# Xingskcs/Distributed-TensorFlow-Examples

Measured on AMD Instinct MI355X. Metric: images/sec (whole node), MNIST CNN sync all-reduce, higher is better.
Workload: dtype bf16; 1 GPU; model=mnist_cnn (conv5x5x32-pool-conv5x5x64-pool-fc1024-dropout-fc10, 3274634 params), global_batch=1024, parallelism=dp1, per_gpu_batch=1024, optimizer=adam (TF1), hip_graph=True, steps_per_graph=4, join_deferred=True, distinct_gpus=1, grad_allreduce=none (1 rank), ranks_seen_by_comm=1

## Files before the change

csrc/bindings/torch_ops.cpp:

```cpp
#include <ATen/ATen.h>
#include <ATen/hip/HIPContext.h>
#include <torch/custom_class.h>
#include <torch/library.h>
#include <algorithm>
#include <cmath>
#include <cstring>
#include <vector>

#include "../kernels/augment.h"
#include "../kernels/conv.h"
#include "../kernels/conv_f32.h"
#include "../kernels/imgconv.h"
#include "../kernels/norm.h"
#include "../kernels/elementwise.h"
#include "../kernels/eval.h"
#include "../kernels/gemm_dense.h"
#include "../kernels/head.h"
#include "../kernels/lstm_seq.h"
#include "../kernels/gradnorm.h"
#include "../kernels/optim.h"
#include "opt_state.h"

using at::Tensor;
using c10::optional;
// ... 271 lines not shown
  a.w = reinterpret_cast<const dtfe::bf16*>(w.data_ptr());
  a.bias = ptr_or_null<float>(bias);
  a.act = (int)act; a.pool = pool;
  a.y = reinterpret_cast<dtfe::bf16*>(y.data_ptr());
  a.argmax = ptr_or_null<uint8_t>(argmax);
  a.relu_mask = ptr_or_null<dtfe::bf16>(relu_mask);
  TORCH_CHECK(w.numel() == N * KH * KW * CS, "imgconv: weight size");
  TORCH_CHECK(y.numel() == B * OH * OW * N / (pool ? 4 : 1), "imgconv: output size");
  a.tstamp = tstamp.has_value() && tstamp->defined() ? reinterpret_cast<uint64_t*>(tstamp->data_ptr()) : nullptr;
  a.bns = bn_src_of(bn_src, (long)B * SH * SW, CS, bn_eps, bn_momentum, bn_save);
  TORCH_CHECK(!a.bns.stats || a.src, "imgconv: BN-on-load needs a plain source");
  a.sc_src = ptr_or_null<dtfe::bf16>(sc_src);
  if (a.sc_src) {
    TORCH_CHECK(sc_stride >= 1 && OH % sc_stride == 0 && OW % sc_stride == 0 && sc_src->dim() == 4 &&
                    sc_src->size(0) == B && sc_src->size(1) == OH / sc_stride && sc_src->size(2) == OW / sc_stride &&
                    sc_src->size(3) >= N,
                "imgconv: shortcut gradient [B][OH/s][OW/s][>= N]");
    a.sc_stride = (int)sc_stride;
    a.sc_C = (int)sc_src->size(3);
  }
  return dtfe::launch_imgconv(a, cur_stream());
}

void conv1_gather_fwd(const Tensor& images, const Tensor& labels_src, int64_t seed, const Tensor& counter,
                      const Tensor& done, const Tensor& labels_dst, const Tensor& x, const Tensor& w,
                      const optional<Tensor>& bias, const Tensor& y, const Tensor& argmax, at::TensorList zero) {
  check_cuda(images, "images");
  TORCH_CHECK(images.scalar_type() == at::kByte && images.dim() == 2 && images.size(1) == 784,
              "conv1_gather_fwd: uint8 [rows][784] dataset");
  TORCH_CHECK(x.scalar_type() == at::kBFloat16 && x.numel() % 784 == 0, "conv1_gather_fwd: bf16 x [B][28][28]");
  dtfe::ImgConvArgs a{};
  a.B = (int)(x.numel() / 784); a.SH = a.SW = 28; a.CS = 1; a.OH = a.OW = 28; a.N = 32;
  a.KH = a.KW = 5; a.stride = 1; a.pad = 2; a.dil = 1;
  a.src = reinterpret_cast<const dtfe::bf16*>(x.data_ptr());
  a.w = reinterpret_cast<const dtfe::bf16*>(w.data_ptr());
  a.bias = ptr_or_null<float>(bias);
  a.act = dtfe::ACT_RELU; a.pool = 1;
  a.y = reinterpret_cast<dtfe::bf16*>(y.data_ptr());
  a.argmax = reinterpret_cast<uint8_t*>(argmax.data_ptr());
  TORCH_CHECK(w.numel() == 32 * 25 && y.numel() == (int64_t)a.B * 14 * 14 * 32 && argmax.numel() == y.numel(),
              "conv1_gather_fwd: MNIST conv1 shapes");
  a.g_src = images.data_ptr<uint8_t>(); a.g_rows = images.size(0); a.g_seed = (uint64_t)seed;
  a.g_counter = counter.data_ptr<int64_t>();
  a.g_done = done.numel() ? reinterpret_cast<uint32_t*>(done.data_ptr()) : nullptr;
  a.g_labels_src = labels_src.data_ptr<int32_t>(); a.g_labels_dst = labels_dst.data_ptr<int32_t>();
  TORCH_CHECK(zero.size() <= 4, "conv1_gather_fwd: at most 4 zero ranges");
  for (const Tensor& z : zero) {
    TORCH_CHECK(z.is_contiguous() && (z.numel() * z.element_size()) % 4 == 0, "conv1_gather_fwd: zero ranges");
    a.zptr[a.nz] = reinterpret_cast<uint32_t*>(z.data_ptr());
    a.zlen[a.nz++] = (long)(z.numel() * z.element_size() / 4);
  }
  TORCH_CHECK(dtfe::launch_conv1_copies_fwd(a, cur_stream()), "conv1_gather_fwd: needs B >= 256");
}

std::vector<int64_t> imgwgrad(const Tensor& src, const optional<Tensor>& dy, const optional<Tensor>& dy_pooled,
                              const optional<Tensor>& dy_argmax, const Tensor& dw, const optional<Tensor>& db,
                              int64_t B, int64_t SH, int64_t SW, int64_t CS, int64_t OH, int64_t OW, int64_t N,
                              int64_t KH, int64_t KW, int64_t stride, int64_t pad, double scale,
                              const optional<Tensor>& ws, int64_t max_blocks, const optional<at::TensorList>& bn_src,
                              double bn_eps, bool defer) {
  check_cuda(src, "src");
  dtfe::ImgWgradArgs a{};
  a.defer_reduce = defer ? 1 : 0;
  a.bns = bn_src_of(bn_src, (long)B * SH * SW, CS, bn_eps, 0.0, false);
  a.max_blocks = (int)max_blocks;
  if (ws.has_value() && ws->defined()) {
    TORCH_CHECK(ws->scalar_type() == at::kFloat && ws->numel() >= dtfe::imgwgrad_ws_floats((int)N, (int)(KH * KW * CS)),
                "imgwgrad: workspace too small (ops.wgrad_ws_floats)");
    a.ws = ws->data_ptr<float>();
  }
  a.B = (int)B; a.SH = (int)SH; a.SW = (int)SW; a.CS = (int)CS; a.OH = (int)OH; a.OW = (int)OW; a.N = (int)N;
  a.KH = (int)KH; a.KW = (int)KW; a.stride = (int)stride; a.pad = (int)pad;
  a.src = reinterpret_cast<const dtfe::bf16*>(src.data_ptr());
  a.dy = ptr_or_null<dtfe::bf16>(dy);
  a.dy_pooled = ptr_or_null<dtfe::bf16>(dy_pooled);
// ... 1076 lines not shown
                  y.size(2) == (x.size(2) + 1) / 2, "bn_relu_pool3: y bf16 / am uint8 [B][ceil(H/2)][ceil(W/2)][C]");
  dtfe::BnArgs a = bn_common(x, stats, 1);
  a.gamma = gamma.data_ptr<float>();
  a.beta = beta.data_ptr<float>();
  a.mean = ptr_or_null<float>(mean);
  a.invstd = ptr_or_null<float>(invstd);
  a.moving_mean = ptr_or_null<float>(moving_mean);
  a.moving_var = ptr_or_null<float>(moving_var);
  a.eps = (float)eps; a.momentum = (float)momentum;
  dtfe::launch_bn_relu_pool3(a, reinterpret_cast<dtfe::bf16*>(y.data_ptr()), am.data_ptr<uint8_t>(), (int)x.size(0),
                             (int)x.size(1), (int)x.size(2), (int)y.size(1), (int)y.size(2), cur_stream());
}

void maxpool3_bwd(const Tensor& dy, const Tensor& am, const Tensor& dx) {
  dtfe::launch_maxpool3_bwd(reinterpret_cast<const dtfe::bf16*>(dy.data_ptr()), am.data_ptr<uint8_t>(),
                            reinterpret_cast<dtfe::bf16*>(dx.data_ptr()), (int)dx.size(0), (int)dx.size(1),
                            (int)dx.size(2), (int)dx.size(3), (int)dy.size(1), (int)dy.size(2), cur_stream());
}

TORCH_LIBRARY(dtfe, m) {
  m.def("conv1_gather_fwd(Tensor images, Tensor labels_src, int seed, Tensor(a!) counter, Tensor(b!) done,"
        " Tensor(c!) labels_dst, Tensor(d!) x, Tensor w, Tensor? bias, Tensor(e!) y, Tensor(f!) argmax,"
        " Tensor(g!)[] zero) -> ()");
  m.def("lstm_seq_fwd(Tensor(a!) xh, Tensor K, Tensor bias, float forget_bias, Tensor(b!) act, Tensor(c!) c,"
        " Tensor(d!) hT, Tensor? xsrc=None, Tensor? ysrc=None, Tensor(e!)? ydst=None, Tensor(f!)? zero0=None,"
        " Tensor(g!)? zero1=None) -> bool");
  m.def("lstm_seq_bwd(Tensor K, Tensor act, Tensor c, Tensor dhT, Tensor(a!) dg, int I, Tensor? dl=None,"
        " Tensor? wo=None) -> bool");
  m.def("lstm_status(bool reset=False) -> int", &lstm_status);
  m.def("lstm_last_split() -> int", &lstm_last_split);
  m.def("bn_stats(Tensor x, Tensor(a!) stats) -> ()");
  m.def("bn_infer(Tensor x, Tensor gamma, Tensor beta, Tensor moving_mean, Tensor moving_var, float eps, int act,"
        " Tensor? res, int rstride, int OH, int OW, Tensor(a!) out) -> ()");
  m.def("bn_apply(Tensor x, Tensor stats, Tensor gamma, Tensor beta, Tensor(a!)? mean, Tensor(b!)? invstd,"
        " Tensor(c!)? moving_mean, Tensor(d!)? moving_var, float eps, float momentum, int act, Tensor? res,"
        " int rstride, int OH, int OW, Tensor(e!) out, Tensor(f!)? mask_out=None, Tensor(g!)[]? res_bn=None) -> ()");
  m.def("bn_bwd_stats(Tensor dy, Tensor? y, Tensor x, Tensor mean, Tensor invstd, Tensor(a!) stats, int act,"
        " Tensor? gamma=None, Tensor? beta=None, Tensor(b!)[]? res_bn=None) -> ()");
  m.def("bn_bwd_apply(Tensor dy, Tensor? y, Tensor x, Tensor mean, Tensor invstd, Tensor gamma, Tensor stats,"
        " int act, Tensor(a!) dx, Tensor(b!)? dres, Tensor(c!)? dgamma, Tensor(d!)? dbeta, Tensor? beta=None) -> ()");
  m.def("shortcut_grad_add(Tensor g, Tensor(a!) dx, int stride) -> ()");
  m.def("gap_fwd(Tensor x, Tensor(a!) y) -> ()");
  m.def("gap_bwd(Tensor dy, Tensor(a!) dx) -> ()");
  m.def("maxpool3_fwd(Tensor x, Tensor(a!) y, Tensor(b!) am) -> ()");
  m.def("maxpool3_bwd(Tensor dy, Tensor am, Tensor(a!) dx) -> ()");
  m.def("bn_relu_pool3(Tensor x, Tensor stats, Tensor gamma, Tensor beta, Tensor(a!)? mean, Tensor(b!)? invstd,"
// ... 84 lines not shown
      " Tensor(b!)? loss_rows, Tensor(c!)? loss_sum, Tensor(d!)? correct, Tensor(e!)? probs) -> ()");
  m.def(
      "gan_loss(Tensor d_real, Tensor d_fake, Tensor(a!) gen_loss, Tensor(b!) disc_loss, Tensor(c!) dz_real_disc,"
      " Tensor(d!) dz_fake_disc, Tensor(e!) dz_fake_gen, float clamp_eps) -> ()");
  m.def("gan_disc_head(Tensor d1, Tensor w, Tensor? b, Tensor(a!)? p, Tensor(b!)? dlog, Tensor(c!)? dlog_g,"
        " Tensor(d!) gw, Tensor(e!)? gb, Tensor(f!) dd1, Tensor(g!) ddf, Tensor(h!) gen_loss, Tensor(i!) disc_loss,"
        " Tensor(j!) ws, float clamp_eps=0.0) -> bool");
  m.def("gan_head_ws_floats(int B, int DH) -> int");
  m.def("epoch_signal(Tensor(a!) ctr) -> ()");
  m.def("mse_sigmoid(Tensor y, Tensor t, Tensor(a!) loss, Tensor(b!) dz, Tensor(c!)? ws=None) -> ()");
  m.def("colsum(Tensor x, int M, int N, int ld, Tensor(a!) db, float scale) -> ()");
  m.def("unpool_f32(Tensor g, Tensor argmax, Tensor(a!) out, int B, int PH, int PW, int C) -> ()");
  m.def("head_xent_f32(Tensor h, Tensor w, Tensor? b, Tensor labels, Tensor(a!) dz, Tensor(b!) dl, Tensor(c!) loss_sum,"
        " Tensor(d!) correct, Tensor(e!)? logits, float scale, float inv_keep, Tensor(f!)? step_counter) -> bool");
  m.def("conv1_wgrad_pooled_f32(Tensor dp, Tensor argmax, Tensor x, Tensor(a!) dw, Tensor(b!)? db, Tensor(c!) ws,"
        " int B, int H, int W, int K, float scale) -> bool");
  m.def("transpose_taps_f32(Tensor input, Tensor(a!) out, int O, int T, int C) -> ()");
  m.def("act_grad(Tensor dy, Tensor y, Tensor(a!) dz, int act) -> ()");
  m.def("bias_act(Tensor x, Tensor? bias, Tensor(a!) out, int act, float keep, int seed, Tensor? counter) -> ()");
}

TORCH_LIBRARY_IMPL(dtfe, CUDA, m) {
  m.impl("conv1_gather_fwd", &conv1_gather_fwd);
  m.impl("lstm_seq_fwd", &lstm_seq_fwd);
  m.impl("lstm_seq_bwd", &lstm_seq_bwd);
  m.impl("bn_stats", &bn_stats);
  m.impl("bn_apply", &bn_apply);
  m.impl("bn_infer", &bn_infer);
  m.impl("bn_bwd_stats", &bn_bwd_stats);
  m.impl("bn_bwd_apply", &bn_bwd_apply);
  m.impl("shortcut_grad_add", &shortcut_grad_add);
  m.impl("gap_fwd", &gap_fwd);
  m.impl("gap_bwd", &gap_bwd);
  m.impl("maxpool3_fwd", &maxpool3_fwd);
  m.impl("maxpool3_bwd", &maxpool3_bwd);
  m.impl("bn_relu_pool3", &bn_relu_pool3);
  m.impl("pool3_bn_bwd", &pool3_bn_bwd);
  m.impl("gemm", &gemm);
  m.impl("conv_fwd", &conv_fwd);
  m.impl("conv_dgrad", &conv_dgrad);
  m.impl("conv_wgrad", &conv_wgrad);
  m.impl("head_xent", &head_xent);
  m.impl("head_wgrad", &head_wgrad);
  m.impl("grad_sumsq", &grad_sumsq);
  m.impl("scale_", &scale_);
  m.impl("eval_metrics", &eval_metrics);
// ... 33 lines not shown
```

csrc/kernels/imgconv.h:

```cpp
#pragma once
#include "bn_chan.h"
#include "common.h"

namespace dtfe {

struct ImgConvArgs {
  int B, SH, SW, CS;
  int OH, OW, N;
  int KH, KW, stride, pad;
  int flip_taps;
  int dil;
  const bf16* src;
  const bf16* src_pooled;
  const uint8_t* src_argmax;
  const bf16* w;
  const float* bias;
  int act, pool;
  bf16* y;
  uint8_t* argmax;
  const bf16* relu_mask;
  const uint8_t* g_src;
  long g_rows;
  uint64_t g_seed;
  int64_t* g_counter;
// ... 19 lines not shown
  int imgs_per_block;
  float* ws;
  int max_blocks;
  int diag;
  BnSrc bns;
  int defer_reduce;
};

struct WpReduceItem {
  const float* ws; float* dw; float* db; float scale; int nblk, plen, MT, CTW, KC, N;
};
constexpr int WP_GROUP_MAX = 32;
void launch_wgrad_reduce_group(const WpReduceItem* it, int n, hipStream_t s);

bool imgconv_supported(int SH, int SW, int CS, int N, int KH, int KW, int stride, int pad);
bool launch_imgconv(const ImgConvArgs& a, hipStream_t s);
bool launch_imgconv_persistent(const ImgConvArgs& a, hipStream_t s, bool* sc_done = nullptr);
bool imgwgrad_supported(const ImgWgradArgs& a);
long imgwgrad_ws_floats(int N, int KC);
void launch_imgwgrad(const ImgWgradArgs& a, hipStream_t s, WpReduceItem& deferred);
bool launch_imgwgrad_persistent(const ImgWgradArgs& a, hipStream_t s, WpReduceItem& deferred);
bool launch_conv1_copies_fwd(const ImgConvArgs& a, hipStream_t s);
bool launch_conv1_copies_wgrad(const ImgWgradArgs& a, hipStream_t s);


void launch_partials_reduce(const float* ws, int nblk, int len, int nw, float* dw, float* db, float scale,
                            hipStream_t s);


__device__ __forceinline__ void unpool4(const u32x4_t pv, const u32x2_t am, u32x4_t (&out)[4]) {
#pragma unroll
  for (int h = 0; h < 2; ++h) {
    const uint32_t lo = am[h] & 0x01010101u, hi = (am[h] >> 1) & 0x01010101u;
    const uint32_t m[4] = {((lo | hi) ^ 0x01010101u) * 0xFFu, (lo & ~hi) * 0xFFu, (hi & ~lo) * 0xFFu,
                           (lo & hi) * 0xFFu};
#pragma unroll
    for (int q = 0; q < 4; ++q) {
      out[q][2 * h] = pv[2 * h] & __builtin_amdgcn_perm(0u, m[q], 0x01010000u);
      out[q][2 * h + 1] = pv[2 * h + 1] & __builtin_amdgcn_perm(0u, m[q], 0x03030202u);
    }
  }
}

}
```

csrc/kernels/imgconv1_copies.hip:

```cpp
#include "imgconv.h"

#include <stdexcept>
#include <type_traits>

namespace dtfe {

namespace {

constexpr int TH = 256;
constexpr int HI = 28;
constexpr int PWD = 48, PRW = 32;
constexpr int CWD = 40;
constexpr int CSZ = PRW * CWD + 8;
constexpr int NCH = 32;
constexpr int XCH = HI * HI / 4;

__device__ __forceinline__ u32x4_t ld16l(const bf16* p) { return *reinterpret_cast<const u32x4_t*>(p); }

template <int B, int E, typename F>
__device__ __forceinline__ void static_for_c1(F&& f) {
  if constexpr (B < E) {
    f(std::integral_constant<int, B>{});
    static_for_c1<B + 1, E>(f);
  }
}

__device__ __forceinline__ void load_img(const bf16* x, long b, u32x2_t& v) {
  if (threadIdx.x < XCH) v = *reinterpret_cast<const u32x2_t*>(x + b * (HI * HI) + threadIdx.x * 4);
}
__device__ __forceinline__ void write_img(bf16* P, const u32x2_t& v) {
  if (threadIdx.x < XCH) {
    const int r = threadIdx.x / 7, c = (threadIdx.x - r * 7) * 4;
    *reinterpret_cast<u32x2_t*>(P + (r + 2) * PWD + c + 4) = v;
  }
}

__device__ __forceinline__ uint32_t shr16(uint32_t lo, uint32_t hi) {
  return (uint32_t)((((uint64_t)hi << 32) | lo) >> 16);
}
template <int S>
__device__ __forceinline__ void build_copies(const bf16* P, bf16* C) {
  constexpr int HALF = (S + 1) / 2;
  const int t = threadIdx.x & 127, r = t >> 2, c8 = (t & 3) * 8;
  const u32x4_t* src = reinterpret_cast<const u32x4_t*>(P + r * PWD + c8);
  uint32_t d[12];
#pragma unroll
  for (int j = 0; j < 3; ++j) {
    const u32x4_t v = src[j];
#pragma unroll
    for (int e = 0; e < 4; ++e) d[4 * j + e] = v[e];
  }
  auto emit = [&](auto sc) {
    constexpr int s = decltype(sc)::value;
    constexpr int e0 = s + 2;
    u32x4_t o;
#pragma unroll
    for (int j = 0; j < 4; ++j) o[j] = (e0 & 1) ? shr16(d[(e0 >> 1) + j], d[(e0 >> 1) + j + 1]) : d[(e0 >> 1) + j];
    *reinterpret_cast<u32x4_t*>(C + s * CSZ + r * CWD + c8) = o;
  };
  if (threadIdx.x < 128) {
    static_for_c1<0, HALF>(emit);
  } else {
    static_for_c1<HALF, S>(emit);
  }
}

template <int ACT>
__global__ __launch_bounds__(TH) void conv1c_fwd_kernel(ImgConvArgs a) {
  __shared__ __attribute__((aligned(16))) bf16 P[PRW * PWD];
  __shared__ __attribute__((aligned(16))) bf16 C[8 * CSZ];
  const int lane = threadIdx.x & 63, wid = threadIdx.x >> 6, g = lane >> 4;
  for (int i = threadIdx.x; i < PRW * PWD / 8; i += TH) reinterpret_cast<u32x4_t*>(P)[i] = u32x4_t{0u, 0u, 0u, 0u};

  bf16x8_t bw[2][2];
  float biasv[2];
#pragma unroll
  for (int nt = 0; nt < 2; ++nt) {
    const int n = nt * 16 + (lane & 15);
    biasv[nt] = a.bias ? a.bias[n] : 0.f;
#pragma unroll
    for (int st = 0; st < 2; ++st) {
      const int kh = st == 0 ? g : 4;
      const bool rowok = st == 0 || g == 0;
      s16x8_t v;
#pragma unroll
      for (int j = 0; j < 8; ++j) v[j] = (short)((rowok && j < 5) ? a.w[n * 25 + kh * 5 + j] : 0);
      bw[nt][st] = __builtin_bit_cast(bf16x8_t, v);
    }
  }

  const int64_t gstep = a.g_src ? *a.g_counter : 0;
  for (int z = 0; z < ((a.diag & 8) ? 0 : a.nz); ++z)
    for (long i = (long)blockIdx.x * TH + threadIdx.x; i < a.zlen[z]; i += (long)gridDim.x * TH) a.zptr[z][i] = 0u;
  auto load = [&](long bb, u32x2_t& v) {
    if (!a.g_src) {
      load_img(a.src, bb, v);
      return;
    }
    const long r = (long)(hash_u32(a.g_seed, (uint64_t)gstep * a.B + bb) % (uint32_t)a.g_rows);
    if (threadIdx.x < XCH) {
      const uint32_t px = *reinterpret_cast<const uint32_t*>(a.g_src + r * (HI * HI) + threadIdx.x * 4);
      const float k = 1.f / 255.f;
      v = u32x2_t{pack_bf16x2((float)(px & 0xffu) * k, (float)((px >> 8) & 0xffu) * k),
                  pack_bf16x2((float)((px >> 16) & 0xffu) * k, (float)(px >> 24) * k)};
      *reinterpret_cast<u32x2_t*>(const_cast<bf16*>(a.src) + bb * (HI * HI) + threadIdx.x * 4) = v;
    }
    if (threadIdx.x == 0 && a.g_labels_dst) a.g_labels_dst[bb] = a.g_labels_src[r];
  };
  u32x2_t xv = {0u, 0u};
  long b = blockIdx.x;
  if (b < a.B) load(b, xv);
  __syncthreads();
  for (; b < a.B; b += gridDim.x) {
    write_img(P, xv);
    __syncthreads();
    if (b + gridDim.x < a.B) load(b + gridDim.x, xv);
    if (!(a.diag & 2)) build_copies<8>(P, C);
    __syncthreads();
    for (int t = wid; t < ((a.diag & 4) ? 0 : 49); t += 4) {
      const int m = t * 16 + (lane & 15), q = m & 3, w = m >> 2;
      const int oy = 2 * (w / 14) + (q >> 1), ox = 2 * (w % 14) + (q & 1);
      const int s = ox & 7;
      const bf16* ab = C + s * CSZ + (ox - s) + oy * CWD;
      const bf16x8_t a0 = __builtin_bit_cast(bf16x8_t, ld16l(ab + g * CWD));
      const bf16x8_t a1 = __builtin_bit_cast(bf16x8_t, ld16l(ab + 4 * CWD));
      f32x4_t acc[2];
#pragma unroll
// ... 197 lines not shown
```

distributed-tensorflow-examples_amd/models/mnist_cnn.py:

```python
from __future__ import annotations

import contextlib

import torch

from .. import ops
from ..optim import FlatParams, Optimizer, OptimizerConfig, VarSpec
from .base import ModelDef, ScaledScalar, StepProgram

IMG, C1, C2, FC, NCLS = 28, 32, 64, 1024, 10
KS = 5


def _normal(std):
    return lambda shape, g: torch.randn(*shape, generator=g) * std


def _zeros(shape, g):
    return torch.zeros(*shape)


def _conv_to_tf(t):
    return t.permute(1, 2, 3, 0).contiguous()

# ... 94 lines not shown
        self.data_ctr = torch.zeros(1, dtype=torch.int64, device=d)
        self.data_done = torch.zeros(1, dtype=torch.int32, device=d)
        self.no_done = torch.zeros(0, dtype=torch.int32, device=d)
        self.g1 = dict(B=B, H=IMG, W=IMG, C=1, Cout=C1, OH=IMG, OW=IMG, KH=KS, KW=KS, stride=1, pad=2)
        self.g2 = dict(B=B, H=14, W=14, C=C1, Cout=C2, OH=14, OW=14, KH=KS, KW=KS, stride=1, pad=2)
        self.ic1 = dict(B=B, SH=IMG, SW=IMG, CS=1, OH=IMG, OW=IMG, N=C1, KH=KS, KW=KS, stride=1, pad=2)
        self.ic2 = dict(B=B, SH=14, SW=14, CS=C1, OH=14, OW=14, N=C2, KH=KS, KW=KS, stride=1, pad=2)
        self.ic2_dgrad = dict(B=B, SH=14, SW=14, CS=C2, OH=14, OW=14, N=C1, KH=KS, KW=KS, stride=1, pad=KS - 1 - 2)
        n = self.names
        P = self.P
        self.w = {k: P.w16[n[k]] for k in ("wc1", "wc2", "wd1", "out")}
        self.wt = {"wc2": P.wt16[n["wc2"]]}
        self.b = {k: P.view(n[k]) for k in ("bc1", "bc2", "bd1", "bout")}
        self.gw = {k: P.gview(n[k]) for k in ("wc1", "wc2", "wd1", "out", "bc1", "bc2", "bd1", "bout")}
        lo1, hi1 = P.range_of([n["out"], n["bout"], n["bd1"], n["wd1"]])
        lo2, hi2 = P.range_of([n["wc2"], n["bc2"], n["wc1"], n["bc1"]])
        self.buckets = [(lo1, hi1), (lo2, hi2)]
        ra = P.range_of([n["out"], n["bout"]])
        rc = P.range_of([n["wc2"], n["bc2"], n["wc1"], n["bc1"]])
        self.accum = [P.grad[ra[0]:ra[1]], P.grad[rc[0]:rc[1]], self.loss_sum, self.correct]
        self.par = self.device.type == "cuda"
        self.c2_blocks = 192
        self.fused_gather = True
        self.late_split = True
        K1 = 7 * 7 * C2
        self.t_fwd = self._glds_tile(self.p2, P.w16[n["wd1"]], B, FC, K1, K1, K1, 19)
        self.t_dgrad = (self._glds_tile(self.dzf, P.w16[n["wd1"]], B, K1, FC, FC, K1, ops.FC_TILE, bmode=ops.RMAJ)
                        or self._glds_tile(self.dzf, P.w16[n["wd1"]], B, K1, FC, FC, K1, 12))
        self.t_wgrad = (self._glds_tile(self.dzf, self.p2, FC, K1 + 1, B, FC, K1, ops.FC_TILE, b_ones_row=K1,
                                        bmode=ops.RMAJ)
                        or self._glds_tile(self.dzf, self.p2, FC, K1 + 1, B, FC, K1, 12, b_ones_row=K1))
        if (self.t_dgrad == ops.FC_TILE) != (self.t_wgrad == ops.FC_TILE):
            self.t_dgrad = self._glds_tile(self.dzf, P.w16[n["wd1"]], B, K1, FC, FC, K1, 12)
            self.t_wgrad = self._glds_tile(self.dzf, self.p2, FC, K1 + 1, B, FC, K1, 12, b_ones_row=K1)
        self.head_gemm = batch > 1024
        self.head_parts = None if self.head_gemm else torch.zeros(2 * ((B + 3) // 4), device=d, dtype=torch.float32)
        self.head_splits = max(1, min(16, B // 128))
        bm, bn = ops.TILE_DIMS[4]
        ntiles = -(-NCLS // bm) * -(-(FC + 1) // bn)
        self.ws_head = (torch.empty(self.head_splits * ntiles * bm * bn, device=d, dtype=torch.float32),
                        torch.zeros(ntiles, device=d, dtype=torch.int32)) if self.head_gemm else None
        self.opt_fc = self.opt_conv = None
        self._late = None
        self.schedule = []
        self.logits = None
        if self.par:
            self.s_c2 = torch.cuda.Stream(device=d)
            self.ws_c2 = torch.empty(ops.wgrad_ws_floats(C2, KS * KS * C1), device=d, dtype=torch.float32)
            self.c2_done = torch.zeros(1, device=d, dtype=torch.int32)
            self.c2_seen = torch.zeros(1, device=d, dtype=torch.int32)
        self.defer_join = False
        self._pending_join = False

    def _glds_tile(self, A, Bm, M, N, K, lda, ldb, tile, b_ones_row=-1, bmode=ops.KMAJ):
        if self.device.type == "cuda" and ops.glds_ok(A, Bm, M, N, K, tile, lda, ldb, b_ones_row=b_ones_row,
                                                      bmode=bmode):
            return tile
        return None

    def forward(self, keep=None, logits=None):
        B = self.B
        keep = self.keep if keep is None else keep
        if self.data is not None and self.device.type == "cuda" and B >= 256 and self.fused_gather:
            ops.require().conv1_gather_fwd(self.data.images, self.data.labels, self.seed + 1, self.data_ctr,
                                           self.no_done, self.labels, self.x, self.w["wc1"], self.b["bc1"],
                                           self.p1, self.a1, self.accum)
        else:
            if self.data is not None:
                ops.gather_rows(self.data.images, self.x.view(B, -1), None, self.data.labels, self.labels,
                                seed=self.seed + 1, counter=self.data_ctr, done=None, zero=self.accum)
            else:
                for t in self.accum:
                    t.zero_()
            ops.imgconv(self.w["wc1"], self.p1, src=self.x, bias=self.b["bc1"], argmax=self.a1, act=ops.ACT_RELU,
                        pool=True, **self.ic1)
        ops.imgconv(self.w["wc2"], self.p2, src=self.p1, bias=self.b["bc2"], argmax=self.a2, act=ops.ACT_RELU,
                    pool=True, **self.ic2)
        K1 = 7 * 7 * C2
        ops.gemm(self.p2, self.w["wd1"], self.h, M=B, N=FC, K=K1, bias=self.b["bd1"], act=ops.ACT_RELU,
                 keep=keep, seed=self.seed + 2, counter=self.data_ctr, tile=self.t_fwd)
        ops.head_xent(self.h, self.w["out"], self.b["bout"], self.labels, self.dzf, self.dl, self.loss_sum,
                      self.correct, logits, scale=1.0 / B, inv_keep=1.0 / keep,
                      step_counter=self.data_ctr if self.data is not None else None,
                      parts=self.head_parts)

    def forward_backward(self):
        B = self.B
        K1 = 7 * 7 * C2
        self.schedule = []
        self.forward()
        main = torch.cuda.current_stream(self.device) if self.par else None
        with ops.gemm_group(self.dzf) as grp:
            self._head_wgrad(grp)
            self._fc1_dgrad(B, K1, grp)
            self._fc1_wgrad(B, K1, grp)
        if self.allreduce is not None:
            self.allreduce.launch(0)
            self.schedule.append("allreduce:0")
        if self.par:
            self.s_c2.wait_stream(main)
# ... 269 lines not shown
```

distributed-tensorflow-examples_amd/ops/__init__.py:

```python
from __future__ import annotations

import contextlib
import functools
import math
import os

import numpy as np
import torch

from ._lib import (ACT_CODES, ACT_NONE, ACT_RELU, ACT_SIGMOID, ACT_TANH, KMAJ, OPT_ADAM, OPT_MOMENTUM,
                   OPT_RMSPROP, OPT_SGD, RMAJ, available, load, require)

__all__ = [
    "gemm", "linear_fwd", "conv_fwd", "conv_dgrad", "conv_wgrad", "head_xent", "apply_gradients", "apply_gradients_group", "opt_state",
    "gather_rows", "uniform_fill", "cast_", "softmax_xent", "gan_loss", "mse_sigmoid", "colsum", "act_grad",
    "bias_act", "ACT_NONE", "ACT_RELU", "ACT_SIGMOID", "ACT_TANH", "ACT_CODES", "KMAJ", "RMAJ", "OPT_SGD",
    "OPT_MOMENTUM", "OPT_ADAM", "OPT_RMSPROP", "available", "load", "require", "pick_tile", "split_workspace",
    "TILE_DIMS", "FC_TILE", "TILE_SMALL", "GEMM_KTILE", "GLDS_TILES", "glds_ok", "ones_page", "bn_stats", "bn_apply", "bn_bwd_stats",
    "bn_bwd_apply", "relu_bits", "shortcut_grad_add",
    "gap_fwd", "gap_bwd", "gemm_group", "seq_stage", "wgrad_tallk", "tallk_ws_floats", "maxpool3_fwd", "maxpool3_bwd", "bn_relu_pool3", "pool3_bn_bwd", "imgconv", "imgwgrad", "hash_u32", "hash_uniform",
    "imgconv_shortcut", "dense_head", "WgradReduces", "conv1_wgrad_pooled_f32",
    "head_xent_f32", "gan_disc_head", "gan_head_ws_floats", "epoch_signal", "grad_norm_plan", "grad_sumsq", "scale_",
    "augment_rows", "augment_draws", "AUG_SALT", "epoch_permutation", "shuffled_rows", "SHUF_SALT", "lr_schedule_spec", "lr_schedule_value", "lr_schedule_pack",
    "eval_metrics", "eval_state", "eval_state_dict", "eval_rows_ref",
# ... 374 lines not shown
        sd = torch.zeros(B, SH * dil, SW * dil, CS)
        sd[:, ::dil, ::dil, :] = s
        s = sd
    wt = w.float().view(N, KH, KW, CS)
    if flip_taps:
        wt = wt.flip(1, 2)
    z = torch.nn.functional.conv2d(s.permute(0, 3, 1, 2), wt.permute(0, 3, 1, 2),
                                   bias.float() if bias is not None else None, stride=stride, padding=pad)
    z = z[:, :, :OH, :OW]
    z = _act_ref(z, act)
    if pool:
        p, idx = _pool_ref(z)
        y.view(-1)[:] = p.permute(0, 2, 3, 1).reshape(-1).to(y.dtype)
        if argmax is not None:
            argmax.view(-1)[:] = idx.permute(0, 2, 3, 1).reshape(-1).to(argmax.dtype)
        return y
    flat = z.permute(0, 2, 3, 1).reshape(-1)
    if relu_mask is not None:
        flat = flat * (relu_mask.reshape(-1).float() > 0)
    y.view(-1)[:] = flat.to(y.dtype)
    return y


def imgconv_shortcut(w, dx, g, sc_stride, *, src, **geom) -> bool:
    if dx.is_cuda:
        k = geom
        return bool(require().imgconv(src, None, None, w, None, dx, None, None, k["B"], k["SH"], k["SW"], k["CS"],
                                      k["OH"], k["OW"], k["N"], k["KH"], k["KW"], k.get("stride", 1), k.get("pad", 0),
                                      True, ACT_NONE, False, k.get("dil", 1), g, sc_stride))
    imgconv(w, dx, src=src, flip_taps=True, **geom)
    shortcut_grad_add(g, dx, sc_stride)
    return True


_WG_WS = {}


def wgrad_ws_floats(N: int, KC: int) -> int:
    MT, CTW = (4, 7) if N > 32 else (2, 9)
    return 256 * max(N * KC + N, 8 * CTW * MT * 256 + (N + 3) // 4 * 4)


def wgrad_workspace(device, numel):
    key = torch.device(device)
    ws = _WG_WS.get(key)
    if ws is None or ws.numel() < numel:
# ... 894 lines not shown
```

Baseline: 5.507 million images/sec.

## Fuse MNIST conv1 gather and conv2 forward into one LDS-resident kernel

Adds a kernel that gathers a sample, runs conv1+ReLU+pool, keeps the pooled output in LDS, then runs conv2+ReLU+pool with MFMA and writes p1, a1, p2 and a2. It replaces the separate conv2 imgconv launch in the forward pass and shares the conv1 helper code through a common header. The aim is to drop one kernel launch and the global round trip of p1 into conv2. The cost is about 160KB of LDS per block, so only one block fits per CU. The grid is fixed at 256 blocks that each walk several images in turn, which may hurt conv2 parallelism compared with the old tiled conv2 kernel.

```diff
diff --git a/csrc/bindings/torch_ops.cpp b/csrc/bindings/torch_ops.cpp
--- a/csrc/bindings/torch_ops.cpp
+++ b/csrc/bindings/torch_ops.cpp
@@ -317,9 +317,10 @@
   return dtfe::launch_imgconv(a, cur_stream());
 }
 
-void conv1_gather_fwd(const Tensor& images, const Tensor& labels_src, int64_t seed, const Tensor& counter,
-                      const Tensor& done, const Tensor& labels_dst, const Tensor& x, const Tensor& w,
-                      const optional<Tensor>& bias, const Tensor& y, const Tensor& argmax, at::TensorList zero) {
+dtfe::ImgConvArgs conv1_gather_args(const Tensor& images, const Tensor& labels_src, int64_t seed, const Tensor& counter,
+                                    const Tensor& done, const Tensor& labels_dst, const Tensor& x, const Tensor& w,
+                                    const optional<Tensor>& bias, const Tensor& y, const Tensor& argmax,
+                                    at::TensorList zero) {
   check_cuda(images, "images");
   TORCH_CHECK(images.scalar_type() == at::kByte && images.dim() == 2 && images.size(1) == 784,
               "conv1_gather_fwd: uint8 [rows][784] dataset");
@@ -345,7 +346,40 @@
     a.zptr[a.nz] = reinterpret_cast<uint32_t*>(z.data_ptr());
     a.zlen[a.nz++] = (long)(z.numel() * z.element_size() / 4);
   }
+  return a;
+}
+
+void conv1_gather_fwd(const Tensor& images, const Tensor& labels_src, int64_t seed, const Tensor& counter,
+                      const Tensor& done, const Tensor& labels_dst, const Tensor& x, const Tensor& w,
+                      const optional<Tensor>& bias, const Tensor& y, const Tensor& argmax, at::TensorList zero) {
+  const dtfe::ImgConvArgs a = conv1_gather_args(images, labels_src, seed, counter, done, labels_dst, x, w, bias, y,
+                                                argmax, zero);
   TORCH_CHECK(dtfe::launch_conv1_copies_fwd(a, cur_stream()), "conv1_gather_fwd: needs B >= 256");
+}
+
+void conv12_gather_fwd(const Tensor& images, const Tensor& labels_src, int64_t seed, const Tensor& counter,
+                       const Tensor& done, const Tensor& labels_dst, const Tensor& x, const Tensor& w,
+                       const optional<Tensor>& bias, const Tensor& y, const Tensor& argmax, at::TensorList zero,
+                       const Tensor& w2, const optional<Tensor>& bias2, const Tensor& p2, const Tensor& a2) {
+  const dtfe::ImgConvArgs a = conv1_gather_args(images, labels_src, seed, counter, done, labels_dst, x, w, bias, y,
+                                                argmax, zero);
+  check_cuda(w2, "w2");
+  check_cuda(p2, "p2");
+  check_cuda(a2, "a2");
+  TORCH_CHECK(w2.scalar_type() == at::kBFloat16 && w2.is_contiguous() && w2.numel() == 64 * 25 * 32,
+              "conv12_gather_fwd: bf16 conv2 weight [64][5*5][32]");
+  TORCH_CHECK(p2.scalar_type() == at::kBFloat16 && p2.is_contiguous() && p2.numel() == (int64_t)a.B * 7 * 7 * 64,
+              "conv12_gather_fwd: bf16 p2 [B][7][7][64]");
+  TORCH_CHECK(a2.scalar_type() == at::kByte && a2.is_contiguous() && a2.numel() == p2.numel(),
+              "conv12_gather_fwd: uint8 a2 [B][7][7][64]");
+  TORCH_CHECK(y.scalar_type() == at::kBFloat16 && argmax.scalar_type() == at::kByte && w.scalar_type() == at::kBFloat16,
+              "conv12_gather_fwd: bf16 p1 / conv1 weight, uint8 a1");
+  if (bias2.has_value() && bias2->defined())
+    TORCH_CHECK(bias2->scalar_type() == at::kFloat && bias2->numel() >= 64, "conv12_gather_fwd: fp32 conv2 bias [64]");
+  TORCH_CHECK(dtfe::launch_conv12_fused_fwd(a, reinterpret_cast<const dtfe::bf16*>(w2.data_ptr()),
+                                            ptr_or_null<float>(bias2), reinterpret_cast<dtfe::bf16*>(p2.data_ptr()),
+                                            a2.data_ptr<uint8_t>(), cur_stream()),
+              "conv12_gather_fwd: needs B >= 256");
 }
 
 std::vector<int64_t> imgwgrad(const Tensor& src, const optional<Tensor>& dy, const optional<Tensor>& dy_pooled,
@@ -1468,6 +1502,9 @@
   m.def("conv1_gather_fwd(Tensor images, Tensor labels_src, int seed, Tensor(a!) counter, Tensor(b!) done,"
         " Tensor(c!) labels_dst, Tensor(d!) x, Tensor w, Tensor? bias, Tensor(e!) y, Tensor(f!) argmax,"
         " Tensor(g!)[] zero) -> ()");
+  m.def("conv12_gather_fwd(Tensor images, Tensor labels_src, int seed, Tensor(a!) counter, Tensor(b!) done,"
+        " Tensor(c!) labels_dst, Tensor(d!) x, Tensor w, Tensor? bias, Tensor(e!) y, Tensor(f!) argmax,"
+        " Tensor(g!)[] zero, Tensor w2, Tensor? bias2, Tensor(h!) p2, Tensor(i!) a2) -> ()");
   m.def("lstm_seq_fwd(Tensor(a!) xh, Tensor K, Tensor bias, float forget_bias, Tensor(b!) act, Tensor(c!) c,"
         " Tensor(d!) hT, Tensor? xsrc=None, Tensor? ysrc=None, Tensor(e!)? ydst=None, Tensor(f!)? zero0=None,"
         " Tensor(g!)? zero1=None) -> bool");
@@ -1598,6 +1635,7 @@
 
 TORCH_LIBRARY_IMPL(dtfe, CUDA, m) {
   m.impl("conv1_gather_fwd", &conv1_gather_fwd);
+  m.impl("conv12_gather_fwd", &conv12_gather_fwd);
   m.impl("lstm_seq_fwd", &lstm_seq_fwd);
   m.impl("lstm_seq_bwd", &lstm_seq_bwd);
   m.impl("bn_stats", &bn_stats);
diff --git a/csrc/kernels/imgconv.h b/csrc/kernels/imgconv.h
--- a/csrc/kernels/imgconv.h
+++ b/csrc/kernels/imgconv.h
@@ -65,6 +65,8 @@
 bool launch_imgwgrad_persistent(const ImgWgradArgs& a, hipStream_t s, WpReduceItem& deferred);
 bool launch_conv1_copies_fwd(const ImgConvArgs& a, hipStream_t s);
 bool launch_conv1_copies_wgrad(const ImgWgradArgs& a, hipStream_t s);
+bool launch_conv12_fused_fwd(const ImgConvArgs& a, const bf16* w2, const float* b2, bf16* p2, uint8_t* a2,
+                             hipStream_t s);
 
 
 void launch_partials_reduce(const float* ws, int nblk, int len, int nw, float* dw, float* db, float scale,
diff --git a/csrc/kernels/imgconv12_fused.hip b/csrc/kernels/imgconv12_fused.hip
--- /dev/null
+++ b/csrc/kernels/imgconv12_fused.hip
@@ -0,0 +1,255 @@
+#include "imgconv.h"
+#include "imgconv1_common.h"
+
+namespace dtfe {
+
+namespace {
+
+using namespace c1;
+
+constexpr int WAVES = 13, THREADS = 64 * WAVES;
+constexpr int CS = 32, KH = 5, KW = 5, LWP = 20, PS = 48, N2 = 64, NT = N2 / 16;
+constexpr int K2 = KH * KW * CS, NK = K2 / 32, KP = K2 + 16;
+constexpr int PH = HI / 2;
+constexpr int LH = PH + KH - 1;
+constexpr int QH = PH / 2, Q2 = QH * QH;
+constexpr int P1N = PH * PH * NCH;
+constexpr int P2N = Q2 * N2;
+constexpr int W_EL = N2 * KP, IMG_EL = LH * LWP * PS;
+constexpr int STAGE_B = P2N * 3, COPIES_B = 8 * CSZ * 2;
+constexpr int UNION_B = COPIES_B > STAGE_B ? COPIES_B : STAGE_B;
+constexpr int P_B = PRW * PWD * 2;
+constexpr int LDS_B = W_EL * 2 + IMG_EL * 2 + UNION_B + P_B;
+static_assert(W_EL * 2 == 104448 && IMG_EL * 2 == 34560 && STAGE_B == 9408 && COPIES_B == 20608 && P_B == 3072,
+              "LDS regions");
+static_assert(LDS_B == 162688 && LDS_B <= 160 * 1024, "LDS budget");
+static_assert(K2 % 32 == 0 && PS >= CS + NCH / 2, "a pixel's pad bytes hold its 32 argmax bytes");
+static_assert((PH * PH + 15) / 16 == WAVES, "one conv2 row tile per wave");
+
+struct Conv12Args {
+  ImgConvArgs c1;
+  const bf16* w2;
+  const float* b2;
+  bf16* p2;
+  uint8_t* a2;
+};
+
+template <int B, int E, typename F>
+__device__ __forceinline__ void static_for(F&& f) {
+  if constexpr (B < E) {
+    f(std::integral_constant<int, B>{});
+    static_for<B + 1, E>(f);
+  }
+}
+
+__device__ __forceinline__ int row_window(int m) {
+  const int t = m >> 4, quad = (m >> 2) & 3;
+  const int w = t * 4 + (quad == 0 ? 0 : quad == 1 ? 2 : quad == 2 ? 3 : 1);
+  return w < Q2 ? w : -1;
+}
+
+__global__ __launch_bounds__(THREADS) void conv12_fwd_kernel(Conv12Args A) {
+  extern __shared__ __attribute__((aligned(16))) bf16 lds[];
+  bf16* wl = lds;
+  bf16* img = wl + W_EL;
+  bf16* C = img + IMG_EL;
+  bf16* sy = C;
+  uint8_t* sa = reinterpret_cast<uint8_t*>(sy + P2N);
+  bf16* P = C + UNION_B / 2;
+  const ImgConvArgs& a = A.c1;
+  const int tid = threadIdx.x, lane = tid & 63, wid = __builtin_amdgcn_readfirstlane(tid >> 6), g = lane >> 4;
+
+  for (int i = tid; i < IMG_EL / 8; i += THREADS) reinterpret_cast<u32x4_t*>(img)[i] = u32x4_t{0u, 0u, 0u, 0u};
+  for (int i = tid; i < PRW * PWD / 8; i += THREADS) reinterpret_cast<u32x4_t*>(P)[i] = u32x4_t{0u, 0u, 0u, 0u};
+
+  const int64_t gstep = *a.g_counter;
+  for (int z = 0; z < a.nz; ++z)
+    for (long i = (long)blockIdx.x * THREADS + tid; i < a.zlen[z]; i += (long)gridDim.x * THREADS) a.zptr[z][i] = 0u;
+
+  uint32_t px = 0u;
+  int32_t lab = 0;
+  auto fetch = [&](long bb) {
+    const long r = (long)(hash_u32(a.g_seed, (uint64_t)gstep * a.B + bb) % (uint32_t)a.g_rows);
+    if (tid < XCH) px = *reinterpret_cast<const uint32_t*>(a.g_src + r * (HI * HI) + tid * 4);
+    if (tid == 0) lab = a.g_labels_src[r];
+  };
+  long b = blockIdx.x;
+  if (b < a.B) fetch(b);
+
+  {
+    constexpr int kc_row = KP / 8, total = N2 * kc_row;
+    static_assert(total <= 8 * THREADS, "one pass");
+    u32x4_t v[8];
+    int off[8];
+#pragma unroll
+    for (int u = 0; u < 8; ++u) {
+      const int i = tid + u * THREADS;
+      const int n = i / kc_row, k = (i - n * kc_row) * 8;
+      off[u] = i < total ? n * KP + k : -1;
+      v[u] = u32x4_t{0u, 0u, 0u, 0u};
+      if (i < total && k < K2) v[u] = *reinterpret_cast<const u32x4_t*>(A.w2 + (long)n * K2 + k);
+    }
+#pragma unroll
+    for (int u = 0; u < 8; ++u)
+      if (off[u] >= 0) *reinterpret_cast<u32x4_t*>(wl + off[u]) = v[u];
+  }
+
+  bf16x8_t bw[2][2];
+  float bias1[2];
+  load_conv1_weights(a.w, a.bias, lane, g, bw, bias1);
+
+  const bf16* wlane = wl + (lane & 15) * KP + 8 * g;
+  float bias2[NT];
+#pragma unroll
+  for (int n = 0; n < NT; ++n) bias2[n] = A.b2 ? A.b2[n * 16 + (lane & 15)] : 0.f;
+  const bf16* abase;
+  {
+    const int m = wid * 16 + (lane & 15), w = row_window(m), q = m & 3;
+    const int oy = 2 * (w / QH) + (q >> 1), ox = 2 * (w % QH) + (q & 1);
+    abase = img + (w >= 0 ? (oy * LWP + ox) * PS : 0) + 8 * g;
+  }
+  const int ppix = row_window(wid * 16 + g * 4);
+
+  __syncthreads();
+  for (; b < a.B; b += gridDim.x) {
+    if (tid < XCH) {
+      const u32x2_t v = px4_to_bf16(px);
+      *reinterpret_cast<u32x2_t*>(const_cast<bf16*>(a.src) + b * (HI * HI) + tid * 4) = v;
+      write_img(P, v);
+    }
+    if (tid == 0 && a.g_labels_dst) a.g_labels_dst[b] = lab;
+    __syncthreads();
+    if (b + gridDim.x < a.B) fetch(b + gridDim.x);
+    build_copies8_by4(P, C);
+    __syncthreads();
+
+    for (int t = wid; t < 49; t += WAVES) {
+      const int m = t * 16 + (lane & 15), q = m & 3, w = m >> 2;
+      const int oy = 2 * (w / 14) + (q >> 1), ox = 2 * (w % 14) + (q & 1);
+      const int s = ox & 7;
+      const bf16* ab = C + s * CSZ + (ox - s) + oy * CWD;
+      const bf16x8_t a0 = __builtin_bit_cast(bf16x8_t, ld16l(ab + g * CWD));
+      const bf16x8_t a1 = __builtin_bit_cast(bf16x8_t, ld16l(ab + 4 * CWD));
+      f32x4_t acc[2];
+#pragma unroll
+      for (int nt = 0; nt < 2; ++nt) {
+        acc[nt] = __builtin_amdgcn_mfma_f32_16x16x32_bf16(a0, bw[nt][0], f32x4_t{0.f, 0.f, 0.f, 0.f}, 0, 0, 0);
+        acc[nt] = __builtin_amdgcn_mfma_f32_16x16x32_bf16(a1, bw[nt][1], acc[nt], 0, 0, 0);
+      }
+      const int wq = t * 4 + g, py = wq / 14, pxx = wq - py * 14;
+      bf16* pp = img + ((py + 2) * LWP + pxx + 2) * PS;
+      uint8_t* pa = reinterpret_cast<uint8_t*>(pp + CS);
+#pragma unroll
+      for (int nt = 0; nt < 2; ++nt) {
+        const f32x4_t v = acc[nt];
+        int am = 0;
+        float mx = v[0];
+#pragma unroll
+        for (int j = 1; j < 4; ++j) if (v[j] > mx) { mx = v[j]; am = j; }
+        const int ch = nt * 16 + (lane & 15);
+        pp[ch] = f2bf(apply_act(mx + bias1[nt], ACT_RELU));
+        pa[ch] = (uint8_t)am;
+      }
+    }
+    __syncthreads();
+
+    {
+      const long ob = b * (long)P1N;
+      for (int i = tid; i < P1N / 8 + P1N / 16; i += THREADS) {
+        const bool isv = i < P1N / 8;
+        const int k = isv ? i : i - P1N / 8;
+        const int pix = isv ? k >> 2 : k >> 1, py = pix / PH, pxx = pix - py * PH;
+        const bf16* pp = img + ((py + 2) * LWP + pxx + 2) * PS;
+        if (isv) {
+          *reinterpret_cast<u32x4_t*>(a.y + ob + k * 8) = *reinterpret_cast<const u32x4_t*>(pp + (k & 3) * 8);
+        } else {
+          *reinterpret_cast<u32x4_t*>(a.argmax + ob + k * 16) =
+              *reinterpret_cast<const u32x4_t*>(reinterpret_cast<const uint8_t*>(pp + CS) + (k & 1) * 16);
+        }
+      }
+    }
+
+    f32x4_t acc[NT];
+#pragma unroll
+    for (int n = 0; n < NT; ++n) acc[n] = f32x4_t{0.f, 0.f, 0.f, 0.f};
+    constexpr int PF = 2;
+    u32x4_t fa[PF + 1], fb[PF + 1][NT];
+    auto fetch_frag = [&](auto sc) {
+      constexpr int st = decltype(sc)::value;
+      constexpr int k0 = 32 * st, tap = k0 / CS, cs = k0 - tap * CS;
+      constexpr int toff = ((tap / KW) * LWP + (tap % KW)) * PS + cs;
+      constexpr int buf = st % (PF + 1);
+      fa[buf] = *reinterpret_cast<const u32x4_t*>(abase + toff);
+#pragma unroll
+      for (int n = 0; n < NT; ++n) fb[buf][n] = *reinterpret_cast<const u32x4_t*>(wlane + n * 16 * KP + k0);
+    };
+    static_for<0, PF>([&](auto sc) { fetch_frag(sc); });
+    static_for<0, NK>([&](auto sc) {
+      constexpr int st = decltype(sc)::value;
+      if constexpr (st + PF < NK) fetch_frag(std::integral_constant<int, st + PF>{});
+      constexpr int buf = st % (PF + 1);
+#pragma unroll
+      for (int n = 0; n < NT; ++n)
+        acc[n] = __builtin_amdgcn_mfma_f32_16x16x32_bf16(__builtin_bit_cast(bf16x8_t, fa[buf]),
+                                                         __builtin_bit_cast(bf16x8_t, fb[buf][n]), acc[n], 0, 0, 0);
+      constexpr int nm = NT, nr = (st + PF < NK) ? 1 + NT : 0;
+      static_for<0, nm>([&](auto ic) {
+        constexpr int i = decltype(ic)::value, r0 = i * nr / nm, r1 = (i + 1) * nr / nm;
+        if constexpr (r1 > r0) __builtin_amdgcn_sched_group_barrier(0x100, r1 - r0, 0);
+        __builtin_amdgcn_sched_group_barrier(0x8, 1, 0);
+      });
+    });
+    if (ppix >= 0) {
+#pragma unroll
+      for (int n = 0; n < NT; ++n) {
+        const int col = n * 16 + (lane & 15);
+        const f32x4_t v = acc[n];
+        int am = 0;
+        float mx = v[0];
+#pragma unroll
+        for (int j = 1; j < 4; ++j) if (v[j] > mx) { mx = v[j]; am = j; }
+        sy[ppix * N2 + col] = f2bf(apply_act(mx + bias2[n], ACT_RELU));
+        sa[ppix * N2 + col] = (uint8_t)am;
+      }
+    }
+    __syncthreads();
+    {
+      constexpr int ny = P2N / 8, na = P2N / 16;
+      const long pb = b * (long)P2N;
+      for (int i = tid; i < ny + na; i += THREADS) {
+        if (i < ny) {
+          *reinterpret_cast<u32x4_t*>(A.p2 + pb + i * 8) = *reinterpret_cast<const u32x4_t*>(sy + i * 8);
+        } else {
+          const int k = i - ny;
+          *reinterpret_cast<u32x4_t*>(A.a2 + pb + k * 16) = *reinterpret_cast<const u32x4_t*>(sa + k * 16);
+        }
+      }
+    }
+  }
+  if (a.g_done && tid == 0) {
+    const uint32_t prev = __hip_atomic_fetch_add(a.g_done, 1u, __ATOMIC_RELAXED, __HIP_MEMORY_SCOPE_AGENT);
+    if (prev == gridDim.x - 1) {
+      __hip_atomic_fetch_add((unsigned long long*)a.g_counter, 1ull, __ATOMIC_RELAXED, __HIP_MEMORY_SCOPE_AGENT);
+      __hip_atomic_store(a.g_done, 0u, __ATOMIC_RELAXED, __HIP_MEMORY_SCOPE_AGENT);
+    }
+  }
+}
+
+}
+
+bool launch_conv12_fused_fwd(const ImgConvArgs& a, const bf16* w2, const float* b2, bf16* p2, uint8_t* a2,
+                             hipStream_t s) {
+  if (a.B < 256 || a.SH != HI || a.SW != HI || a.CS != 1 || a.OH != HI || a.OW != HI || a.N != NCH || a.KH != 5 ||
+      a.KW != 5 || a.stride != 1 || a.pad != 2)
+    return false;
+  if (!a.src || !a.pool || a.flip_taps || a.dil > 1 || a.relu_mask || a.act != ACT_RELU) return false;
+  if (!a.g_src || !a.g_counter || !a.g_labels_src || !a.y || !a.argmax || !w2 || !p2 || !a2) return false;
+  Conv12Args A{a, w2, b2, p2, a2};
+  A.c1.diag = 0;
+  const int grid = a.B < 256 ? a.B : 256;
+  (void)hipFuncSetAttribute((const void*)conv12_fwd_kernel, hipFuncAttributeMaxDynamicSharedMemorySize, LDS_B);
+  hipLaunchKernelGGL(conv12_fwd_kernel, dim3(grid), dim3(THREADS), LDS_B, s, A);
+  return true;
+}
+
+}
diff --git a/csrc/kernels/imgconv1_common.h b/csrc/kernels/imgconv1_common.h
--- /dev/null
+++ b/csrc/kernels/imgconv1_common.h
@@ -0,0 +1,119 @@
+#pragma once
+#include "common.h"
+
+#include <type_traits>
+
+namespace dtfe {
+namespace c1 {
+
+constexpr int TH = 256;
+constexpr int HI = 28;
+constexpr int PWD = 48, PRW = 32;
+constexpr int CWD = 40;
+constexpr int CSZ = PRW * CWD + 8;
+constexpr int NCH = 32;
+constexpr int XCH = HI * HI / 4;
+
+__device__ __forceinline__ u32x4_t ld16l(const bf16* p) { return *reinterpret_cast<const u32x4_t*>(p); }
+
+template <int B, int E, typename F>
+__device__ __forceinline__ void static_for_c1(F&& f) {
+  if constexpr (B < E) {
+    f(std::integral_constant<int, B>{});
+    static_for_c1<B + 1, E>(f);
+  }
+}
+
+__device__ __forceinline__ void load_img(const bf16* x, long b, u32x2_t& v) {
+  if (threadIdx.x < XCH) v = *reinterpret_cast<const u32x2_t*>(x + b * (HI * HI) + threadIdx.x * 4);
+}
+__device__ __forceinline__ void write_img(bf16* P, const u32x2_t& v) {
+  if (threadIdx.x < XCH) {
+    const int r = threadIdx.x / 7, c = (threadIdx.x - r * 7) * 4;
+    *reinterpret_cast<u32x2_t*>(P + (r + 2) * PWD + c + 4) = v;
+  }
+}
+
+__device__ __forceinline__ u32x2_t px4_to_bf16(uint32_t px) {
+  const float k = 1.f / 255.f;
+  return u32x2_t{pack_bf16x2((float)(px & 0xffu) * k, (float)((px >> 8) & 0xffu) * k),
+                 pack_bf16x2((float)((px >> 16) & 0xffu) * k, (float)(px >> 24) * k)};
+}
+
+__device__ __forceinline__ uint32_t shr16(uint32_t lo, uint32_t hi) {
+  return (uint32_t)((((uint64_t)hi << 32) | lo) >> 16);
+}
+template <int S>
+__device__ __forceinline__ void build_copies(const bf16* P, bf16* C) {
+  constexpr int HALF = (S + 1) / 2;
+  const int t = threadIdx.x & 127, r = t >> 2, c8 = (t & 3) * 8;
+  const u32x4_t* src = reinterpret_cast<const u32x4_t*>(P + r * PWD + c8);
+  uint32_t d[12];
+#pragma unroll
+  for (int j = 0; j < 3; ++j) {
+    const u32x4_t v = src[j];
+#pragma unroll
+    for (int e = 0; e < 4; ++e) d[4 * j + e] = v[e];
+  }
+  auto emit = [&](auto sc) {
+    constexpr int s = decltype(sc)::value;
+    constexpr int e0 = s + 2;
+    u32x4_t o;
+#pragma unroll
+    for (int j = 0; j < 4; ++j) o[j] = (e0 & 1) ? shr16(d[(e0 >> 1) + j], d[(e0 >> 1) + j + 1]) : d[(e0 >> 1) + j];
+    *reinterpret_cast<u32x4_t*>(C + s * CSZ + r * CWD + c8) = o;
+  };
+  if (threadIdx.x < 128) {
+    static_for_c1<0, HALF>(emit);
+  } else {
+    static_for_c1<HALF, S>(emit);
+  }
+}
+
+__device__ __forceinline__ void build_copies8_by4(const bf16* P, bf16* C) {
+  if (threadIdx.x >= 512) return;
+  const int t = threadIdx.x & 127, r = t >> 2, c8 = (t & 3) * 8;
+  const u32x4_t* src = reinterpret_cast<const u32x4_t*>(P + r * PWD + c8);
+  uint32_t d[12];
+#pragma unroll
+  for (int j = 0; j < 3; ++j) {
+    const u32x4_t v = src[j];
+#pragma unroll
+    for (int e = 0; e < 4; ++e) d[4 * j + e] = v[e];
+  }
+  auto emit = [&](auto sc) {
+    constexpr int s = decltype(sc)::value;
+    constexpr int e0 = s + 2;
+    u32x4_t o;
+#pragma unroll
+    for (int j = 0; j < 4; ++j) o[j] = (e0 & 1) ? shr16(d[(e0 >> 1) + j], d[(e0 >> 1) + j + 1]) : d[(e0 >> 1) + j];
+    *reinterpret_cast<u32x4_t*>(C + s * CSZ + r * CWD + c8) = o;
+  };
+  switch (threadIdx.x >> 7) {
+    case 0: static_for_c1<0, 2>(emit); break;
+    case 1: static_for_c1<2, 4>(emit); break;
+    case 2: static_for_c1<4, 6>(emit); break;
+    default: static_for_c1<6, 8>(emit); break;
+  }
+}
+
+__device__ __forceinline__ void load_conv1_weights(const bf16* w, const float* bias, int lane, int g,
+                                                   bf16x8_t (&bw)[2][2], float (&biasv)[2]) {
+#pragma unroll
+  for (int nt = 0; nt < 2; ++nt) {
+    const int n = nt * 16 + (lane & 15);
+    biasv[nt] = bias ? bias[n] : 0.f;
+#pragma unroll
+    for (int st = 0; st < 2; ++st) {
+      const int kh = st == 0 ? g : 4;
+      const bool rowok = st == 0 || g == 0;
+      s16x8_t v;
+#pragma unroll
+      for (int j = 0; j < 8; ++j) v[j] = (short)((rowok && j < 5) ? w[n * 25 + kh * 5 + j] : 0);
+      bw[nt][st] = __builtin_bit_cast(bf16x8_t, v);
+    }
+  }
+}
+
+}
+}
diff --git a/csrc/kernels/imgconv1_copies.hip b/csrc/kernels/imgconv1_copies.hip
--- a/csrc/kernels/imgconv1_copies.hip
+++ b/csrc/kernels/imgconv1_copies.hip
@@ -1,4 +1,5 @@
 #include "imgconv.h"
+#include "imgconv1_common.h"
 
 #include <stdexcept>
 #include <type_traits>
@@ -7,63 +8,7 @@
 
 namespace {
 
-constexpr int TH = 256;
-constexpr int HI = 28;
-constexpr int PWD = 48, PRW = 32;
-constexpr int CWD = 40;
-constexpr int CSZ = PRW * CWD + 8;
-constexpr int NCH = 32;
-constexpr int XCH = HI * HI / 4;
-
-__device__ __forceinline__ u32x4_t ld16l(const bf16* p) { return *reinterpret_cast<const u32x4_t*>(p); }
-
-template <int B, int E, typename F>
-__device__ __forceinline__ void static_for_c1(F&& f) {
-  if constexpr (B < E) {
-    f(std::integral_constant<int, B>{});
-    static_for_c1<B + 1, E>(f);
-  }
-}
-
-__device__ __forceinline__ void load_img(const bf16* x, long b, u32x2_t& v) {
-  if (threadIdx.x < XCH) v = *reinterpret_cast<const u32x2_t*>(x + b * (HI * HI) + threadIdx.x * 4);
-}
-__device__ __forceinline__ void write_img(bf16* P, const u32x2_t& v) {
-  if (threadIdx.x < XCH) {
-    const int r = threadIdx.x / 7, c = (threadIdx.x - r * 7) * 4;
-    *reinterpret_cast<u32x2_t*>(P + (r + 2) * PWD + c + 4) = v;
-  }
-}
-
-__device__ __forceinline__ uint32_t shr16(uint32_t lo, uint32_t hi) {
-  return (uint32_t)((((uint64_t)hi << 32) | lo) >> 16);
-}
-template <int S>
-__device__ __forceinline__ void build_copies(const bf16* P, bf16* C) {
-  constexpr int HALF = (S + 1) / 2;
-  const int t = threadIdx.x & 127, r = t >> 2, c8 = (t & 3) * 8;
-  const u32x4_t* src = reinterpret_cast<const u32x4_t*>(P + r * PWD + c8);
-  uint32_t d[12];
-#pragma unroll
-  for (int j = 0; j < 3; ++j) {
-    const u32x4_t v = src[j];
-#pragma unroll
-    for (int e = 0; e < 4; ++e) d[4 * j + e] = v[e];
-  }
-  auto emit = [&](auto sc) {
-    constexpr int s = decltype(sc)::value;
-    constexpr int e0 = s + 2;
-    u32x4_t o;
-#pragma unroll
-    for (int j = 0; j < 4; ++j) o[j] = (e0 & 1) ? shr16(d[(e0 >> 1) + j], d[(e0 >> 1) + j + 1]) : d[(e0 >> 1) + j];
-    *reinterpret_cast<u32x4_t*>(C + s * CSZ + r * CWD + c8) = o;
-  };
-  if (threadIdx.x < 128) {
-    static_for_c1<0, HALF>(emit);
-  } else {
-    static_for_c1<HALF, S>(emit);
-  }
-}
+using namespace c1;
 
 template <int ACT>
 __global__ __launch_bounds__(TH) void conv1c_fwd_kernel(ImgConvArgs a) {
@@ -100,9 +45,7 @@
     const long r = (long)(hash_u32(a.g_seed, (uint64_t)gstep * a.B + bb) % (uint32_t)a.g_rows);
     if (threadIdx.x < XCH) {
       const uint32_t px = *reinterpret_cast<const uint32_t*>(a.g_src + r * (HI * HI) + threadIdx.x * 4);
-      const float k = 1.f / 255.f;
-      v = u32x2_t{pack_bf16x2((float)(px & 0xffu) * k, (float)((px >> 8) & 0xffu) * k),
-                  pack_bf16x2((float)((px >> 16) & 0xffu) * k, (float)(px >> 24) * k)};
+      v = px4_to_bf16(px);
       *reinterpret_cast<u32x2_t*>(const_cast<bf16*>(a.src) + bb * (HI * HI) + threadIdx.x * 4) = v;
     }
     if (threadIdx.x == 0 && a.g_labels_dst) a.g_labels_dst[bb] = a.g_labels_src[r];
diff --git a/distributed-tensorflow-examples_amd/models/mnist_cnn.py b/distributed-tensorflow-examples_amd/models/mnist_cnn.py
--- a/distributed-tensorflow-examples_amd/models/mnist_cnn.py
+++ b/distributed-tensorflow-examples_amd/models/mnist_cnn.py
@@ -140,6 +140,7 @@
         self.par = self.device.type == "cuda"
         self.c2_blocks = 192
         self.fused_gather = True
+        self.fused_conv12 = True
         self.late_split = True
         K1 = 7 * 7 * C2
         self.t_fwd = self._glds_tile(self.p2, P.w16[n["wd1"]], B, FC, K1, K1, K1, 19)
@@ -179,7 +180,12 @@
     def forward(self, keep=None, logits=None):
         B = self.B
         keep = self.keep if keep is None else keep
-        if self.data is not None and self.device.type == "cuda" and B >= 256 and self.fused_gather:
+        fused = self.data is not None and self.device.type == "cuda" and B >= 256 and self.fused_gather
+        if fused and self.fused_conv12:
+            ops.conv12_gather_fwd(self.data.images, self.data.labels, self.seed + 1, self.data_ctr, self.no_done,
+                                  self.labels, self.x, self.w["wc1"], self.b["bc1"], self.p1, self.a1, self.accum,
+                                  self.w["wc2"], self.b["bc2"], self.p2, self.a2)
+        elif fused:
             ops.require().conv1_gather_fwd(self.data.images, self.data.labels, self.seed + 1, self.data_ctr,
                                            self.no_done, self.labels, self.x, self.w["wc1"], self.b["bc1"],
                                            self.p1, self.a1, self.accum)
@@ -192,8 +198,9 @@
                     t.zero_()
             ops.imgconv(self.w["wc1"], self.p1, src=self.x, bias=self.b["bc1"], argmax=self.a1, act=ops.ACT_RELU,
                         pool=True, **self.ic1)
-        ops.imgconv(self.w["wc2"], self.p2, src=self.p1, bias=self.b["bc2"], argmax=self.a2, act=ops.ACT_RELU,
-                    pool=True, **self.ic2)
+        if not (fused and self.fused_conv12):
+            ops.imgconv(self.w["wc2"], self.p2, src=self.p1, bias=self.b["bc2"], argmax=self.a2, act=ops.ACT_RELU,
+                        pool=True, **self.ic2)
         K1 = 7 * 7 * C2
         ops.gemm(self.p2, self.w["wd1"], self.h, M=B, N=FC, K=K1, bias=self.b["bd1"], act=ops.ACT_RELU,
                  keep=keep, seed=self.seed + 2, counter=self.data_ctr, tile=self.t_fwd)
diff --git a/distributed-tensorflow-examples_amd/ops/__init__.py b/distributed-tensorflow-examples_amd/ops/__init__.py
--- a/distributed-tensorflow-examples_amd/ops/__init__.py
+++ b/distributed-tensorflow-examples_amd/ops/__init__.py
@@ -420,6 +420,13 @@
     return y
 
 
+def conv12_gather_fwd(images, labels_src, seed, counter, done, labels_dst, x, w1, b1, p1, a1, zero, w2, b2, p2, a2):
+    if not p2.is_cuda:
+        raise RuntimeError("conv12_gather_fwd: GPU only (the CPU path runs gather_rows and imgconv)")
+    require().conv12_gather_fwd(images, labels_src, seed, counter, done, labels_dst, x, w1, b1, p1, a1, list(zero),
+                                w2, b2, p2, a2)
+
+
 def imgconv_shortcut(w, dx, g, sc_stride, *, src, **geom) -> bool:
     if dx.is_cuda:
         k = geom
```

New measurement: 5.613 million images/sec (median of 6 runs). +1.9%, better.
